# nanoporetech/tombo

Hardware: NVIDIA H100
Metric: resquiggle_reads_per_sec (higher is better)
Workload: dtype f64

## Files before the change

### include/tombo_b200.h

```cpp
#ifndef TOMBO_B200_H
#define TOMBO_B200_H
#include <stdint.h>

#ifdef __cplusplus
extern "C" {
#endif

#define TB2_ABI_VERSION 1

enum {
    TB2_OK = 0,
    TB2_ERR_FEWER_CPTS = 1,
    TB2_ERR_BEYOND_BANDWIDTH = 2,
    TB2_ERR_ADAPTIVE_BEYOND_SIGNAL = 3,
    TB2_ERR_NOT_ENOUGH_DEL_SIGNAL = 4,
    TB2_ERR_TOO_MANY_DELS = 5,
    TB2_ERR_INVALID_SEG = 6,
    TB2_ERR_ZERO_LEN_SEG = 7,
    TB2_ERR_NEG_SEG = 8,
    TB2_ERR_SEG_PAST_END = 9,
    TB2_ERR_START_TOO_FAR = 10,
    TB2_ERR_MASKED_TOO_FEW = 11,
    TB2_ERR_READ_TOO_SHORT_START = 12,
    TB2_ERR_MAP_TOO_SHORT_START = 13,
    TB2_ERR_POOR_START_MATCH = 14,
    TB2_ERR_DISCORDANT_LEN = 15,
    TB2_ERR_OPEN_PORE = 16,
    TB2_ERR_NO_RAW = 17,
    TB2_ERR_TOO_MUCH_SIGNAL = 18,
    TB2_ERR_SEG_COUNT = 19,
    TB2_ERR_THEIL_SEN_ZERO = 20,
    TB2_ERR_INVALID_START_PATH = 21,
    TB2_ERR_UNEXPECTED = 100,
    TB2_ERR_CUDA = 200,
    TB2_ERR_INVALID_ARG = 201,
    TB2_ERR_CAPACITY = 202,
    TB2_ERR_INVALID_SEQ = 203
};

typedef struct tb2_params {
    double match_evalue, skip_pen;
    int64_t bandwidth;
    double max_half_z_score;
    int64_t running_stat_width, min_obs_per_base, raw_min_obs_per_base,
        mean_obs_per_event;
    double z_shift, stay_pen;
    int64_t use_t_test_seg;
    int64_t band_bound_thresh, start_bw, start_save_bw, start_n_bases;
} tb2_params;

typedef struct tb2_scale_values {
    double shift, scale, lower_lim, upper_lim, outlier_thresh;
} tb2_scale_values;

typedef struct tb2_policy {
    double outlier_thresh;
    int64_t max_raw_cpts;
    double min_event_to_seq_ratio;
    double sig_match_thresh;
    int64_t max_scaling_iters;
    int64_t is_rna;
    int64_t skip_seq_scaling;
    double const_scale;
    uint32_t subsample_seed;
    uint32_t rescue;
} tb2_policy;

typedef struct tb2_ctx tb2_ctx;

int tb2_abi_version(void);
int tb2_device_count(void);
int tb2_ctx_create(int device, tb2_ctx **out);
void tb2_ctx_destroy(tb2_ctx *ctx);
const char *tb2_status_message(int status);
const char *tb2_last_error(tb2_ctx *ctx);
int64_t tb2_launch_count(tb2_ctx *ctx);
int tb2_last_timing(tb2_ctx *ctx, double *out4);

void *tb2_host_alloc(size_t bytes);
void tb2_host_free(void *p);

int tb2_set_model(tb2_ctx *ctx, const double *means, const double *sds,
                  int kmer_width, int central_pos);
int tb2_set_alt_model(tb2_ctx *ctx, const double *alt_means, int kmer_width);

int tb2_new_means(tb2_ctx *ctx, const double *sig, int64_t n_sig,
                  const int64_t *segs, int64_t n_segs, double *means_out);
int tb2_new_mean_stds(tb2_ctx *ctx, const double *sig, int64_t n_sig,
                      const int64_t *segs, int64_t n_segs, double *means_out,
                      double *sds_out);
int tb2_normalize_raw_signal(tb2_ctx *ctx, const double *raw, int64_t n,
                             int norm_type, double outlier_thresh,
                             double const_scale, const tb2_scale_values *sv_in,
                             double *norm_out, tb2_scale_values *sv_out);
int tb2_identify_stalls(tb2_ctx *ctx, const double *raw, int64_t n, int64_t *ints_out,
                        int64_t cap, int64_t *n_out);
int tb2_valid_cpts_w_cap(tb2_ctx *ctx, const double *sig, int64_t n,
                         int64_t min_base_obs, int64_t running_stat_width,
                         int64_t num_cpts, int t_test, int64_t *cpts_out,
                         int *read_status);
int tb2_banded_forward_pass(tb2_ctx *ctx, const double *z,
                            const int64_t *event_starts, int64_t n_bases,
                            int64_t bw, double skip_pen, double stay_pen,
                            double *fwd_out, int64_t *tb_out);
int tb2_banded_traceback(tb2_ctx *ctx, const int64_t *tb,
                         const int64_t *event_starts, int64_t n_bases,
                         int64_t bw, int64_t band_pos,
                         int64_t band_boundary_thresh, int64_t *seq_poss_out,
                         int *read_status);
int tb2_adaptive_banded_forward_pass(
    tb2_ctx *ctx, double *fwd, int64_t *tb, int64_t *event_starts,
    int64_t n_bases, int64_t bw, const double *event_means, int64_t n_events,
    const double *ref_means, const double *ref_sds, double z_shift,
    double skip_pen, double stay_pen, int64_t start_seq_pos,
    double mask_fill_z_score, int do_winsorize_z, double max_half_z_score,
    int *read_status);
int tb2_theil_sen(tb2_ctx *ctx, double prev_shift, double prev_scale,
                  const double *event_means, const double *model_means,
                  int64_t n, uint32_t subsample_key, double *out4,
                  int *read_status);

int tb2_find_adaptive_base_assignment(
    tb2_ctx *ctx, const int64_t *valid_cpts, int64_t n_cpts,
    const double *event_means, const tb2_params *params,
    const double *ref_means, const double *ref_sds, int64_t n_bases,
    double sig_match_thresh, int64_t *segs_out, int64_t *read_start_rel_to_raw,
    int64_t *dbg, int *read_status);
int tb2_find_static_base_assignment(tb2_ctx *ctx, const double *event_means,
                                    int64_t n_events, const double *ref_means,
                                    const double *ref_sds, int64_t n_bases,
                                    const tb2_params *params, int64_t *read_tb_out,
                                    int *read_status);
int tb2_find_seq_start_in_events(tb2_ctx *ctx, const double *event_means,
                                 int64_t n_events, const double *ref_means,
                                 const double *ref_sds, int64_t n_ref,
                                 const tb2_params *params, int64_t num_bases,
                                 int64_t num_events, int check_score,
                                 double sig_match_thresh, int64_t *start_loc,
                                 double *events_per_base, int *read_status);
int tb2_debug_last_assignment(tb2_ctx *ctx, int64_t n_bases, int64_t *starts_out,
                              int64_t *read_tb_out);
int tb2_debug_div_check(tb2_ctx *ctx, uint64_t seed, int blocks, int per_thread,
                        uint64_t *mismatches, double *example4);
int tb2_debug_counters(tb2_ctx *ctx, unsigned long long *out8, int reset);
int tb2_resolve_skipped_bases_with_raw(
    tb2_ctx *ctx, const int64_t *segs, int64_t n_bases, const double *ref_means,
    const double *ref_sds, const double *norm_signal, int64_t n_norm,
    const tb2_params *params, int64_t max_raw_cpts, int64_t *segs_out,
    int *read_status);

int tb2_resquiggle_batch(
    tb2_ctx *ctx, int64_t n_reads, const void *raw, int raw_dtype,
    const int64_t *raw_off, const uint8_t *seq, const int64_t *seq_off,
    const tb2_params *params, const tb2_params *save_params,
    const tb2_policy *policy, int64_t *segs, int64_t *read_start_rel_to_raw,
    tb2_scale_values *scale_out, double *sig_match_score, double *norm_mean,
    double *norm_signal, int32_t *status, int32_t *n_iters, int32_t *flags);

int tb2_pipeline_chunks(int sm_count, int64_t n_reads, int64_t *starts_out, int cap);

int tb2_batch_upload(tb2_ctx *ctx, int64_t n_reads, const void *raw, int raw_dtype,
                     const int64_t *raw_off, const uint8_t *seq,
                     const int64_t *seq_off, const tb2_params *params,
                     const tb2_policy *policy);
int tb2_batch_set_read_inputs(tb2_ctx *ctx, const tb2_scale_values *sv_in,
                              const int64_t *stall_ints, const int64_t *stall_off);
int tb2_batch_compute(tb2_ctx *ctx, const tb2_params *params,
                      const tb2_params *save_params, const tb2_policy *policy,
                      int want_norm_signal);
int tb2_batch_download(tb2_ctx *ctx, int64_t *segs, int64_t *read_start_rel_to_raw,
                       tb2_scale_values *scale_out, double *sig_match_score,
                       double *norm_mean, double *norm_signal, int32_t *status,
                       int32_t *n_iters, int32_t *flags);

int tb2_alt_model_llr_batch(
    tb2_ctx *ctx, int64_t n_reads, const double *norm_mean,
    const int64_t *mean_off, const uint8_t *seq, const int64_t *seq_off,
    const int64_t *read_start, int alt_base_code, int use_standard_llhr,
    double scale_factor, double height_factor, double height_power,
    double *llr_out, int64_t *pos_out, int64_t *site_off);

int tb2_calc_llh_ratio_windows(tb2_ctx *ctx, int mode, int64_t n_sites, int kmer_width,
                               const double *means, const double *ref_means,
                               const double *alt_means, const double *var_a,
                               const double *var_b, double scale_factor,
                               double height_factor, double height_power,
                               double *llr_out);

int tb2_timer_start(tb2_ctx *ctx);
int tb2_timer_stop(tb2_ctx *ctx, double *ms_out);

int tb2_batch_alt_llr(tb2_ctx *ctx, const int64_t *read_start, int alt_base_code,
                      int use_standard_llhr, double scale_factor, double height_factor,
                      double height_power, int64_t *n_sites_total);
int tb2_batch_llr_download(tb2_ctx *ctx, double *llr_out, int64_t *pos_out, int64_t *site_off);

int tb2_region_stats_begin(tb2_ctx *ctx, int64_t reg_start, int64_t reg_len);
int tb2_region_stats_add(tb2_ctx *ctx, int64_t n, const double *stats, const int64_t *pos,
                         double single_read_thresh, double lower_thresh, int stat_type);
int tb2_region_stats_add_batch_llr(tb2_ctx *ctx, double single_read_thresh,
                                   double lower_thresh, int stat_type);
int tb2_region_counts_get(tb2_ctx *ctx, int32_t *counts);
int tb2_region_counts_set(tb2_ctx *ctx, const int32_t *counts);
int tb2_region_stats_finalize(tb2_ctx *ctx, double unmod_count, double mod_count, int64_t cap,
                              int64_t *pos_out, double *frac_out, double *damp_frac_out,
                              int64_t *cov_out, int64_t *valid_cov_out, int64_t *n_out);

int tb2_window_fisher_pvals(tb2_ctx *ctx, int64_t n_segs, const double *means,
                            const double *ref_means, const double *ref_sds,
                            const int64_t *seg_off, int64_t fm_offset, int final_clamp,
                            double *pvals_out);
int tb2_de_novo_read_stats_batch(tb2_ctx *ctx, int64_t n_reads, const double *norm_mean,
                                 const int64_t *mean_off, const uint8_t *seq,
                                 const int64_t *seq_off, const int64_t *read_start,
                                 int64_t fm_offset, double *pvals_out, int64_t *pos_out,
                                 int64_t *stat_off);

int tb2_group_reg_stats(tb2_ctx *ctx, int64_t reg_start, int64_t reg_len,
                        int64_t n_samp, const double *samp_levels, const int64_t *samp_off,
                        const int64_t *samp_start, int64_t n_ctrl, const double *ctrl_levels,
                        const int64_t *ctrl_off, const int64_t *ctrl_start, int test,
                        int return_stat, int64_t min_test_reads, int64_t fm_offset, int64_t cap,
                        int64_t *pos_out, double *stat_out, int64_t *cov_out,
                        int64_t *ctrl_cov_out, int64_t *n_out);
int tb2_reads_ref_levels(tb2_ctx *ctx, int64_t reg_start, int64_t reg_len, int64_t n_reads,
                         const double *levels, const int64_t *off, const int64_t *start,
                         int64_t min_test_reads, int est_mean, const double *prior_means,
                         const double *prior_sds, double mean_prior_weight,
                         double sd_prior_weight, double *means_out, double *sds_out,
                         int64_t *cov_out);

#ifdef __cplusplus
}
#endif
#endif
```

### tombo_b200/csrc/stage_kernels.cu

```cuda
#include "stage_kernels.cuh"

static inline int grid1d(int n, int bs) { return (n + bs - 1) / bs; }

int tb2_launch_prep(tb2_ctx *ctx, const BatchView &b, const void *raw_dev, int raw_dtype,
                    int is_rna, long long, long long)
{
    if (raw_dtype == 0)
        k_prep<double><<<b.n_reads, ST_THREADS, 0, ctx->stream>>>(
            b, (const double *)raw_dev, is_rna, ctx->model_means.as<double>(),
            ctx->model_sds.as<double>());
    else
        k_prep<short><<<b.n_reads, ST_THREADS, 0, ctx->stream>>>(
            b, (const short *)raw_dev, is_rna, ctx->model_means.as<double>(),
            ctx->model_sds.as<double>());
    TB2_CHECK_LAUNCH(ctx);
    return TB2_OK;
}

int tb2_launch_start_attempt(tb2_ctx *ctx, const BatchView &b, int attempt)
{
    k_start_attempt<<<grid1d(b.n_reads, 256), 256, 0, ctx->stream>>>(b, attempt);
    TB2_CHECK_LAUNCH(ctx);
    return TB2_OK;
}

int tb2_launch_begin_call(tb2_ctx *ctx, const BatchView &b, const tb2_params &p,
                          const StagePolicy &pol)
{
    k_begin_call<<<grid1d(b.n_reads, 256), 256, 0, ctx->stream>>>(b, p, pol);
    TB2_CHECK_LAUNCH(ctx);
    return TB2_OK;
}

int tb2_launch_end_call(tb2_ctx *ctx, const BatchView &b, int max_iters)
{
    k_end_call<<<grid1d(b.n_reads, 256), 256, 0, ctx->stream>>>(b, max_iters);
    TB2_CHECK_LAUNCH(ctx);
    return TB2_OK;
}

int tb2_launch_count_active(tb2_ctx *ctx, const BatchView &b, int *dev_counter)
{
    TB2_CUDA_TRY(ctx, cudaMemsetAsync(dev_counter, 0, 2 * sizeof(int), ctx->stream));
    k_count_active<<<grid1d(b.n_reads, 256), 256, 0, ctx->stream>>>(b, dev_counter);
    TB2_CHECK_LAUNCH(ctx);
    return TB2_OK;
}

int tb2_launch_normalize(tb2_ctx *ctx, const BatchView &b, const StagePolicy &pol, int first_call)
{
    k_normalize<<<b.n_reads, ST_THREADS, 0, ctx->stream>>>(b, pol, first_call);
    TB2_CHECK_LAUNCH(ctx);
    return TB2_OK;
}

int tb2_launch_cpts(tb2_ctx *ctx, const BatchView &b, const tb2_params &p, int on_raw)
{
    if (!p.use_t_test_seg) {
        k_cumsum<<<(b.n_reads + CS_WARPS - 1) / CS_WARPS, CS_WARPS * 32, 0, ctx->stream>>>(b, on_raw);
        TB2_CHECK_LAUNCH(ctx);
    }
    const long long nw = (b.max_raw + 32) / 32;
    long long words = (4 + std::max(0, (int)p.min_obs_per_base - 1)) * nw;
    if (words * 4 > 48 * 1024) words = 0;
    k_cpts<<<b.n_reads, ST_THREADS, (size_t)words * 4, ctx->stream>>>(b, p, on_raw, (int)words);
    TB2_CHECK_LAUNCH(ctx);
    return TB2_OK;
}

int tb2_launch_rna_scale(tb2_ctx *ctx, const BatchView &b, const StagePolicy &pol)
{
    k_rna_scale<<<b.n_reads, ST_THREADS, 0, ctx->stream>>>(b, pol);
    TB2_CHECK_LAUNCH(ctx);
    return TB2_OK;
}

int tb2_launch_event_means(tb2_ctx *ctx, const BatchView &b)
{
    k_event_means<<<b.n_reads, ST_THREADS, 0, ctx->stream>>>(b);
    TB2_CHECK_LAUNCH(ctx);
    return TB2_OK;
}

int tb2_launch_stalls(tb2_ctx *ctx, const BatchView &b)
{
    k_stalls<<<b.n_reads, ST_THREADS, 0, ctx->stream>>>(b);
    TB2_CHECK_LAUNCH(ctx);
    return TB2_OK;
}

int tb2_launch_resolve(tb2_ctx *ctx, const BatchView &b, const tb2_params &p,
                       const StagePolicy &pol, size_t cap)
{
    enum { SLOT_RAWDP = 73, SLOT_CNT2 = 74, SLOT_RAWBIG = 75 };
    const int warps_per_block = 4;
    int grid = ctx->sm_count * 8;
    const int max_useful = (b.n_reads + warps_per_block - 1) / warps_per_block;
    if (grid > max_useful) grid = max_useful > 0 ? max_useful : 1;
    const size_t slots = (size_t)grid * warps_per_block;
    TB2_CUDA_TRY(ctx, ctx->pool[SLOT_RAWDP].reserve(slots * cap * sizeof(double)));
    TB2_CUDA_TRY(ctx, ctx->pool[SLOT_CNT2].reserve(16));
    TB2_CUDA_TRY(ctx, cudaMemsetAsync(ctx->pool[SLOT_CNT2].p, 0, 16, ctx->stream));
    const unsigned long long big_cap = std::min<unsigned long long>(
        (2ULL << 30) / 8, std::max<unsigned long long>((64ULL << 20) / 8, 24ULL * 64ULL * (unsigned long long)std::max(1, b.max_raw)));
    TB2_CUDA_TRY(ctx, ctx->pool[SLOT_RAWBIG].reserve((size_t)big_cap * sizeof(double)));
    k_resolve<<<grid, warps_per_block * 32, 0, ctx->stream>>>(
        b, p, pol, ctx->pool[SLOT_RAWDP].as<double>(), cap, ctx->pool[SLOT_CNT2].as<int>(),
        ctx->pool[SLOT_RAWBIG].as<double>(), big_cap,
        (unsigned long long *)(ctx->pool[SLOT_CNT2].as<int>() + 2));
    TB2_CHECK_LAUNCH(ctx);
    return TB2_OK;
}

int tb2_launch_base_means(tb2_ctx *ctx, const BatchView &b)
{
    k_base_means<<<b.n_reads, ST_THREADS, 0, ctx->stream>>>(b);
    TB2_CHECK_LAUNCH(ctx);
    return TB2_OK;
}

int tb2_launch_theil_sen(tb2_ctx *ctx, const BatchView &b, const StagePolicy &pol, int first_call)
{
    const size_t smem = sizeof(TsSmem);
    TB2_CUDA_TRY(ctx, cudaFuncSetAttribute(k_theil_sen, cudaFuncAttributeMaxDynamicSharedMemorySize,
                                           (int)smem));
    k_theil_sen<<<b.n_reads, ST_THREADS, smem, ctx->stream>>>(b, pol, first_call);
    TB2_CHECK_LAUNCH(ctx);
    return TB2_OK;
}

int tb2_launch_finalize(tb2_ctx *ctx, const BatchView &b, const StagePolicy &pol, int first_call,
                        double *norm_mean_out, double *norm_signal_out)
{
    k_finalize<<<b.n_reads, ST_THREADS, 0, ctx->stream>>>(b, pol, first_call, norm_mean_out,
                                                          norm_signal_out);
    TB2_CHECK_LAUNCH(ctx);
    return TB2_OK;
}

extern "C" int tb2_debug_counters(tb2_ctx *ctx, unsigned long long *out8, int reset)
{
    int rc = tb2_use(ctx);
    if (rc) return rc;
    if (!out8) return TB2_ERR_INVALID_ARG;
    TB2_CUDA_TRY(ctx, cudaStreamSynchronize(ctx->stream));
    TB2_CUDA_TRY(ctx, cudaMemcpyFromSymbol(out8, g_tb2_counters, 64));
    if (reset) {
        unsigned long long z[8] = {0};
        TB2_CUDA_TRY(ctx, cudaMemcpyToSymbol(g_tb2_counters, z, 64));
    }
    return TB2_OK;
}
```

### tombo_b200/csrc/stage_kernels.cuh

```cuda
#pragma once
#include "batch.h"
#include "select.cuh"

#define ST_THREADS TB2_SEL_THREADS

__device__ __forceinline__ bool rd_active(const ReadState &s) { return s.active && s.status == TB2_OK; }

template <class T>
__global__ void __launch_bounds__(ST_THREADS)
k_prep(BatchView b, const T *raw, int is_rna, const double *kmeans, const double *ksds)
{
    const int r = blockIdx.x;
    const long long ro = b.raw_off[r];
    const int n = (int)(b.raw_off[r + 1] - ro);
    for (int i = threadIdx.x; i < n; i += ST_THREADS)
        b.rawf[ro + i] = (double)raw[ro + (is_rna ? n - 1 - i : i)];
    const long long so = b.seq_off[r], bo = b.base_off[r];
    const int nb = (int)(b.base_off[r + 1] - bo);
    const int K = b.kmer_width;
    int bad = 0;
    for (int i = threadIdx.x; i < nb; i += ST_THREADS) {
        int code = 0;
        for (int j = 0; j < K; ++j) {
            const int c = b.seq[so + i + j];
// ... 692 lines not shown
        for (int i = lane; i <= nb; i += 32) out[i] = segs[i];
        __syncwarp();
        const int n_norm = segs[nb];
        if (lane == 0) s.n_norm = n_norm;
        const double *norm = b.norm + b.raw_off[r] + s.rsrtr;
        const double *rm = b.rm + bo, *rs = b.rs + bo;
        int *ws = b.starts + bo, *we = b.read_tb + bo + r;
        const int n_segs = nb + 1;
        const int m = (int)p.raw_min_obs_per_base;
        int nw = 0, st = TB2_OK;
#define TOO_SMALL(a, z) ((double)(segs[z] - segs[a]) <= ((double)(((z) - (a) + 1) * m)) * EXTRA_SIG_FACTOR)
#define MERGE_TRIM() do { \
            int mm = 0; \
            for (int k = 0; k < nw; ++k) { \
                if (mm > 0 && ws[k] < we[mm - 1]) we[mm - 1] = we[k]; \
                else { ws[mm] = ws[k]; we[mm] = we[k]; ++mm; } } \
            nw = mm; \
            if (ws[0] < 0) ws[0] = 0; \
            if (we[nw - 1] > n_segs - 1) we[nw - 1] = n_segs - 1; } while (0)
        if (lane == 0) {
            for (int d = 0; d < nb; ++d) {
                if (segs[d + 1] - segs[d] != 0) continue;
                if (nw > 0 && d < we[nw - 1] + DEL_FIX_WINDOW) we[nw - 1] = d + DEL_FIX_WINDOW + 1;
                else { ws[nw] = d - DEL_FIX_WINDOW; we[nw] = d + DEL_FIX_WINDOW + 1; ++nw; }
            }
            if (nw > 0) {
                MERGE_TRIM();
                int expanded = 0;
                for (int it = 0; it < MAX_DEL_FIX_WINDOW - DEL_FIX_WINDOW; ++it) {
                    expanded = 0;
                    for (int k = 0; k < nw; ++k)
                        if (TOO_SMALL(ws[k], we[k])) { expanded = 1; ws[k] -= 1; we[k] += 1; }
                    if (!expanded) break;
                    MERGE_TRIM();
                }
                if (expanded)
                    for (int k = 0; k < nw; ++k)
                        if (TOO_SMALL(ws[k], we[k])) { st = TB2_ERR_NOT_ENOUGH_DEL_SIGNAL; break; }
                if (st == TB2_OK && pol.max_raw_cpts >= 0) {
                    int mx = 0;
                    for (int k = 0; k < nw; ++k) mx = max(mx, we[k] - ws[k]);
                    if (mx > pol.max_raw_cpts) st = TB2_ERR_TOO_MANY_DELS;
                }
            }
        }
        nw = __shfl_sync(TB2_FULL_MASK, nw, 0);
        st = __shfl_sync(TB2_FULL_MASK, st, 0);
        if (nw == 0) continue;
        __syncwarp();
        for (int k = 0; k < nw && st == TB2_OK; ++k) {
            const int a = ws[k], z = we[k], n_ev = z - a;
            const int sig_start = segs[a], sig_len = segs[z] - segs[a];
            if (sig_start < 0 || sig_start + sig_len > n_norm) { st = TB2_ERR_UNEXPECTED; break; }
            RawCtx c;
            c.sig = norm + sig_start; c.rm = rm + a; c.rs = rs + a;
            c.n_ev = n_ev; c.m = m;
            c.L = sig_len - (n_ev - 1) * m;
            c.winsor = !isnan(p.max_half_z_score);
            c.mhz = c.winsor ? p.max_half_z_score : 0.0;
            if (c.L < 1) { st = TB2_ERR_UNEXPECTED; break; }
            const size_t need = (size_t)n_ev * c.L + 3 * (size_t)c.L + 8;
            unsigned long long woff = 0;
            if (need > cap) {
                if (lane == 0) woff = atomicAdd(big_used, (unsigned long long)need) + 1ULL;
                woff = __shfl_sync(TB2_FULL_MASK, woff, 0);
                if (woff - 1ULL + need > big_cap) { st = TB2_ERR_CAPACITY; break; }
            }
            double *win = woff ? big_pool + (woff - 1ULL) : scr;
            c.fwd = win;
            c.cs = win + (size_t)n_ev * c.L;
            c.ld0 = (int *)(c.cs + 2 * (size_t)c.L);
            c.ld1 = c.ld0 + c.L;
            if (n_ev < 2) { st = TB2_ERR_UNEXPECTED; break; }
            if (m == 1) raw_forward_wf(c);
            else raw_fill_z(c);
            if (lane == 0) {
                st = (m == 1) ? TB2_OK : raw_window(c, out + a + 1);
                if (st == TB2_OK) st = raw_traceback_rows(c, out + a + 1);
                if (st == TB2_OK) for (int i = 0; i < n_ev - 1; ++i) out[a + 1 + i] += sig_start;
            }
            st = __shfl_sync(TB2_FULL_MASK, st, 0);
            __syncwarp();
        }
        if (lane != 0) continue;
        if (st == TB2_OK) {
            for (int i = 0; i < nb; ++i) if (out[i + 1] - out[i] < 1) { st = TB2_ERR_ZERO_LEN_SEG; break; }
            if (st == TB2_OK && out[0] < 0) st = TB2_ERR_NEG_SEG;
            if (st == TB2_OK && out[nb] > n_norm) st = TB2_ERR_SEG_PAST_END;
        }
        if (st != TB2_OK) s.status = st;
    }
}

__global__ void __launch_bounds__(ST_THREADS) k_base_means(BatchView b)
{
    const int r = blockIdx.x;
    const ReadState &s = b.st[r];
    if (!rd_active(s)) return;
    const long long bo = b.base_off[r];
    const int nb = (int)(b.base_off[r + 1] - bo);
    const double *norm = b.norm + b.raw_off[r] + s.rsrtr;
    const int *segs = b.segs + bo + r;
    for (int i = threadIdx.x; i < nb; i += ST_THREADS) {
        const int a = segs[i], z = segs[i + 1];
        double acc = 0;
        for (int k = a; k < z; ++k) acc += norm[k];
        b.bm[bo + i] = acc / (double)(z - a);
    }
}

__device__ unsigned long long g_tb2_counters[8];

#define TS_MAX 1000
#define TS_BINS 2048
#define TS_BUF 2048

#define TS_ABINS 4096

#define TS_PAD 1024

struct TsSmem {
    double ev[TS_PAD], md[TS_PAD];
    float4 pt[TS_PAD];
    union {
        unsigned int hist[TS_ABINS + 2];
        double buf[TS_BUF];
    };
    unsigned int nbuf, nout, b1, b2, below, maxabs_bits;
    int ok;
};

__device__ __forceinline__ double ts_slope(const TsSmem &t, int i, int j)
{
    return (t.ev[i] == t.ev[j]) ? 1000.0 : (t.md[i] - t.md[j]) / (t.ev[i] - t.ev[j]);
}

template <class Fn>
__device__ __forceinline__ void ts_for_pairs(int n, Fn fn)
{
    const int half = (n + 1) / 2;
    for (int c = threadIdx.x; c < half; c += ST_THREADS) {
        const int j0 = c, j1 = n - 1 - c;
        for (int i = 0; i < j0; ++i) fn(i, j0);
        if (j1 != j0) for (int i = 0; i < j1; ++i) fn(i, j1);
    }
}

template <class Fn>
__device__ __forceinline__ void ts_for_cols(int n, Fn fn)
{
    const int half = (n + 1) / 2;
    for (int c = threadIdx.x; c < half; c += ST_THREADS) {
        const int j0 = c, j1 = n - 1 - c;
        fn(j0);
        if (j1 != j0) fn(j1);
    }
}

__device__ __forceinline__ void ts_pair_of(long long s, int n, int *pi, int *pj)
{
    double disc = (double)(2 * n - 1) * (double)(2 * n - 1) - 8.0 * (double)s;
    int i = (int)(((double)(2 * n - 1) - sqrt(disc)) / 2.0);
    if (i < 0) i = 0;
    auto row_start = [&](int q) { return (long long)q * (2 * n - q - 1) / 2; };
    while (i > 0 && row_start(i) > s) --i;
    while (row_start(i + 1) <= s) ++i;
    *pi = i;
    *pj = (int)(s - row_start(i)) + i + 1;
}


#define TS_SBINS 1024
#define TS_SAMPLES 2048
#define TS_LIST 4096
#define TS_MAX_PHASES 600

__device__ long long ts_sort_count(double **ka, double **kb, unsigned short **pa, unsigned short **pb,
                                   int P, SelectSmem &sm)
{
    const int tid = threadIdx.x;
    unsigned int inv = 0;
    for (int w = 1; w < P; w <<= 1) {
        const double *src = *ka; const unsigned short *sp = *pa;
        double *dst = *kb; unsigned short *dp = *pb;
        for (int p = tid; p < P; p += ST_THREADS) {
            const int base = p & ~(2 * w - 1), mid = base + w;
            const double key = src[p];
            int lo, hi;
            if (p < mid) {
                lo = mid; hi = mid + w;
                while (lo < hi) { const int m = (lo + hi) >> 1; if (src[m] < key) lo = m + 1; else hi = m; }
                dst[p + (lo - mid)] = key; dp[p + (lo - mid)] = sp[p];
            } else {
                lo = base; hi = mid;
                while (lo < hi) { const int m = (lo + hi) >> 1; if (src[m] <= key) lo = m + 1; else hi = m; }
                const int le = lo - base;
                dst[base + (p - mid) + le] = key; dp[base + (p - mid) + le] = sp[p];
                inv += (unsigned int)(w - le);
            }
        }
        __syncthreads();
        double *tk = *ka; *ka = *kb; *kb = tk;
        unsigned short *tp = *pa; *pa = *pb; *pb = tp;
    }
    return (long long)tb2_block_sum(inv, sm);
}

__device__ long long ts_sweep(unsigned short *perm, const double *q, int n, unsigned int *list,
                              unsigned int *n_list, SelectSmem &sm)
{
    const int tid = threadIdx.x;
    unsigned int swaps = 0;
    int quiet = 0;
    for (int ph = 0; ph < TS_MAX_PHASES; ++ph) {
        int any = 0;
        for (int p = 2 * tid + (ph & 1); p + 1 < n; p += 2 * ST_THREADS) {
            const unsigned short x = perm[p], y = perm[p + 1];
            if (q[x] > q[y]) {
                perm[p] = y; perm[p + 1] = x;
                ++swaps; any = 1;
                if (list) {
                    const unsigned int slot = atomicAdd(n_list, 1u);
                    if (slot < TS_LIST) list[slot] = ((unsigned int)min(x, y) << 16) | (unsigned int)max(x, y);
                }
            }
        }
        any = __syncthreads_or(any);
        quiet = any ? 0 : quiet + 1;
        if (quiet >= 2) {
#ifdef TS_DEBUG
            if (tid == 0) atomicAdd(&g_tb2_counters[7], (unsigned long long)(ph + 1));
#endif
            return (long long)tb2_block_sum(swaps, sm);
        }
    }
    tb2_block_sum(swaps, sm);
    return -1;
}

__device__ bool ts_gaps_ok(const unsigned short *perm, const double *q, const double *ev, int n, double g)
{
    int bad = 0;
    for (int p = threadIdx.x; p + 1 < n; p += ST_THREADS) {
        const int x = perm[p], y = perm[p + 1];
        bad |= !(q[y] - q[x] > g) && (ev[x] != ev[y]);
    }
    return !__syncthreads_or(bad);
}

__global__ void __launch_bounds__(ST_THREADS, 4)
k_theil_sen(BatchView b, StagePolicy pol, int first_call)
{
    TB2_DYN_SMEM(unsigned char, ts_raw);
    TsSmem &t = *reinterpret_cast<TsSmem *>(ts_raw);
    __shared__ SelectSmem sm;
    const int r = b.order ? b.order[blockIdx.x] : blockIdx.x;
    ReadState &s = b.st[r];
    if (!rd_active(s)) return;
    const int tid = threadIdx.x;
    if (first_call && pol.skip_seq_scaling) {
        if (tid == 0) { s.changed = 0; s.shc = 0.0; s.scc = 1.0; }
        return;
    }
    const long long bo = b.base_off[r];
    const int nb = (int)(b.base_off[r + 1] - bo);
    const double *bm = b.bm + bo, *rm = b.rm + bo;
    int n = nb;
    if (nb > TS_MAX) {
        n = TS_MAX;
        const unsigned int key = pol.literal_key
            ? pol.subsample_seed
            : tb2_subsample_key(pol.subsample_seed, (unsigned int)(r + pol.read_index_base),
                                (unsigned int)s.calls);
        for (int i = tid; i < n; i += ST_THREADS) {
            const int k = tb2_perm_index(i, nb, key);
            t.ev[i] = bm[k]; t.md[i] = rm[k];
        }
    } else {
        for (int i = tid; i < n; i += ST_THREADS) { t.ev[i] = bm[i]; t.md[i] = rm[i]; }
    }
    __syncthreads();
    const long long Np = (long long)n * (n - 1) / 2;
    if (Np <= 0) { if (tid == 0) s.status = TB2_ERR_UNEXPECTED; return; }
    if (tid == 0) atomicAdd(&g_tb2_counters[0], 1ULL);
    const bool even = (Np % 2) == 0;
    const long long k1 = even ? Np / 2 - 1 : Np / 2;
    double v1 = 0, v2 = 0;
    bool have = false;
    const int hs = n / 2;
    double lo = 0, hi = 0;
    if (hs >= 16) {
        for (int i = tid; i < hs; i += ST_THREADS) t.buf[i] = ts_slope(t, i, i + hs);
        __syncthreads();
        double d0;
        auto f_samp = [&](int i) { return t.buf[i]; };
        tb2_block_select2(f_samp, PredAll(), hs, (int)(hs * 0.30), false, &lo, &d0, sm);
        tb2_block_select2(f_samp, PredAll(), hs, (int)(hs * 0.70), false, &hi, &d0, sm);
    }
    {
        int P = 2;
        while (P < n) P <<= 1;
        for (int i = n + tid; i < P; i += ST_THREADS) { t.ev[i] = __longlong_as_double(0x7ff0000000000000LL); t.md[i] = 0.0; }
        __syncthreads();
        for (int k = 2; k <= P; k <<= 1) {
            for (int jj = k >> 1; jj > 0; jj >>= 1) {
                for (int idx = tid; idx < (P >> 1); idx += ST_THREADS) {
                    const int a = ((idx & ~(jj - 1)) << 1) | (idx & (jj - 1)), c = a | jj;
                    const double ea = t.ev[a], ec = t.ev[c];
                    const double ma = t.md[a], mc = t.md[c];
                    const bool gt = (ea > ec) || (ea == ec && ma > mc);
                    const bool ne = (ea != ec) || (ma != mc);
                    if (ne && (gt == ((a & k) == 0))) {
                        t.ev[a] = ec; t.ev[c] = ea;
                        t.md[a] = mc; t.md[c] = ma;
                    }
                }
                __syncthreads();
            }
        }
    }
    if (hs >= 16 && n >= 128 && hi > lo && hi < 1000.0) {
        double *qa = reinterpret_cast<double *>(t.pt), *qb = qa + TS_PAD;
        unsigned short *pa = reinterpret_cast<unsigned short *>(t.buf + (TS_BUF - 512)), *pb = pa + TS_PAD;
        unsigned int *list = reinterpret_cast<unsigned int *>(qb);
        static_assert(TS_LIST * 4 <= TS_PAD * 8 + (TS_BUF - 512) * 8, "pair list overlaps the id arrays");
        bool ok;
        double M;
        const int n_samples = (int)min(8192LL, max(2048LL, Np / 24));
        {
            int bad = 0;
            double mx = 0.0;
            for (int i = tid; i < n; i += ST_THREADS) {
                const double e = t.ev[i], m = t.md[i];
                if (!(fabs(e) < 1e300) || !(fabs(m) < 1e300)) bad = 1;
                if (i + 1 < n && !(t.ev[i + 1] >= e)) bad = 1;
                mx = fmax(mx, fmax(fabs(e), fabs(m)));
            }
            ok = !__syncthreads_or(bad);
#ifdef TS_DEBUG
            if (!ok && tid == 0) { int c = 0; for (int i = 0; i + 1 < n; ++i) if (!(t.ev[i + 1] > t.ev[i])) { if (c++ < 3) printf("  ev order: i=%d %.17g %.17g\n", i, t.ev[i], t.ev[i + 1]); } }
#endif
            unsigned long long mk = (unsigned long long)__double_as_longlong(mx);
            mk = ~tb2_block_min_u64(~mk, sm);
            M = fmax(1.0, __longlong_as_double((long long)mk));
        }
        const float lo_f = (float)lo, hi_f = (float)hi;
        const float w_f = (hi_f - lo_f) / (float)TS_SBINS;
        ok = ok && (w_f > 0.0f) && isfinite(w_f);
        if (ok) {
            for (int i = tid; i < TS_SBINS + 2; i += ST_THREADS) t.hist[i] = 0;
            __syncthreads();
            const float inv_w = 1.0f / w_f;
            for (int q = tid; q < n_samples; q += ST_THREADS) {
                const uint32_t h1 = tb2_mix32((uint32_t)q * 2654435761u + 17u), h2 = tb2_mix32(h1 ^ 0x9E3779B9u);
                const int i = (int)(((unsigned long long)h1 * (unsigned long long)n) >> 32);
                int j = i + 1 + (int)(((unsigned long long)h2 * (unsigned long long)(n - 1)) >> 32);
                if (j >= n) j -= n;
                const double de = t.ev[i] - t.ev[j];
                const float sa = __fdividef((float)(t.md[i] - t.md[j]), (float)de);
                int bin = 0;
                if (sa >= hi_f || de == 0.0) bin = TS_SBINS + 1;
                else if (sa >= lo_f) bin = min(TS_SBINS - 1, (int)((sa - lo_f) * inv_w)) + 1;
                atomicAdd(&t.hist[bin], 1u);
            }
            __syncthreads();
            const int per = (TS_SBINS + 2 + ST_THREADS - 1) / ST_THREADS;
            const int q0 = min(TS_SBINS + 2, tid * per), q1 = min(TS_SBINS + 2, q0 + per);
            unsigned int mine = 0;
            for (int q = q0; q < q1; ++q) mine += t.hist[q];
            const int lane = tid & 31, warp = tid >> 5;
            unsigned int inc = mine;
#pragma unroll
            for (int off = 1; off < 32; off <<= 1) {
                const unsigned int o = __shfl_up_sync(TB2_FULL_MASK, inc, off);
                if (lane >= off) inc += o;
            }
            if (lane == 31) sm.warp_tot[warp] = inc;
            __syncthreads();
            unsigned int run = inc - mine;
            for (int q = 0; q < warp; ++q) run += sm.warp_tot[q];
            for (int q = q0; q < q1; ++q) { run += t.hist[q]; t.hist[q] = run; }
            __syncthreads();
        }
        auto pick = [&](double frac, int *bsel) -> bool {
            const double tf = frac * (double)n_samples;
            if (!(tf > (double)t.hist[0]) || !(tf < (double)t.hist[TS_SBINS])) return false;
            const unsigned int target = (unsigned int)tf;
            int blo = 1, bhi = TS_SBINS;
            while (blo < bhi) { const int m = (blo + bhi) >> 1; if (t.hist[m] >= target) bhi = m; else blo = m + 1; }
            *bsel = blo;
            return true;
        };
        auto thr = [&](int bsel) { return (double)lo_f + (double)w_f * (double)bsel; };
        const long long kT = even ? k1 + 1 : k1;
        const double sig = 0.5 / sqrt((double)n_samples);
        const double ppm = (double)Np / (double)n_samples;
        int bL = 0, bH1 = 0, bH2 = 0;
        long long invL = 0, inv1 = 0, inv2 = 0;
        if (ok) ok = pick((double)k1 / (double)Np - 3.0 * sig, &bL);
        if (ok) {
            const double TL = thr(bL);
            const double gL = 1e-12 * M * (1.0 + fabs(TL));
            int P = 2;
            while (P < n) P <<= 1;
            for (int i = tid; i < P; i += ST_THREADS) {
                qa[i] = (i < n) ? __fma_rn(-TL, t.ev[i], t.md[i]) : __longlong_as_double(0x7ff0000000000000LL);
                pa[i] = (unsigned short)i;
            }
            __syncthreads();
            double *ka = qa, *kb = qb;
            unsigned short *ia = pa, *ib = pb;
            invL = ts_sort_count(&ka, &kb, &ia, &ib, P, sm);
            int bad = 0;
            for (int p2 = tid; p2 + 1 < n; p2 += ST_THREADS)
                bad |= !(ka[p2 + 1] - ka[p2] > gL) && (t.ev[ia[p2]] != t.ev[ia[p2 + 1]]);
            ok = !__syncthreads_or(bad);
            if (ia != pa) for (int i = tid; i < n; i += ST_THREADS) pa[i] = ia[i];
            __syncthreads();
            ok = ok && invL <= k1;
        }
        bH1 = bL; inv1 = invL;
        for (int stage = 0; ok && stage < 5; ++stage) {
            const double D = (double)(k1 - inv1);
            const double rest = fmax(3.0 * sqrt(D * ppm), 150.0);
            if (D <= rest + 250.0 || D + 3.0 * sqrt(D * ppm) + 300.0 <= 0.8 * TS_LIST) break;
            const double delta = (double)inv1 / (double)Np - (double)t.hist[bH1] / (double)n_samples;
            int bn;
            if (!pick(((double)k1 - rest) / (double)Np - delta, &bn) || bn <= bH1) break;
            const double T1 = thr(bn);
            for (int i = tid; i < n; i += ST_THREADS) qa[i] = __fma_rn(-T1, t.ev[i], t.md[i]);
            __syncthreads();
            const long long sw = ts_sweep(pa, qa, n, nullptr, nullptr, sm);
            ok = sw >= 0 && ts_gaps_ok(pa, qa, t.ev, n, 1e-12 * M * (1.0 + fabs(T1)));
            bH1 = bn; inv1 += sw;
            ok = ok && inv1 <= k1;
#ifdef TS_DEBUG
            if (tid == 0) printf("  stage %d: D=%.0f aimed rest %.0f -> got rest %lld (swaps %lld)\n", stage, D, rest, k1 - inv1, sw);
#endif
        }
        if (ok) {
            const double D = (double)(kT - inv1);
            const double over = fmax(3.0 * sqrt(fmax(D, 1.0) * ppm), 150.0);
            const double delta = (double)inv1 / (double)Np - (double)t.hist[bH1] / (double)n_samples;
            ok = pick(((double)kT + over) / (double)Np - delta, &bH2) && bH2 > bH1;
            if (ok) {
                const double T2 = thr(bH2);
                for (int i = tid; i < n; i += ST_THREADS) qa[i] = __fma_rn(-T2, t.ev[i], t.md[i]);
                if (tid == 0) t.nbuf = 0;
                __syncthreads();
                const long long sw = ts_sweep(pa, qa, n, list, &t.nbuf, sm);
                ok = sw >= 0 && sw <= TS_LIST && ts_gaps_ok(pa, qa, t.ev, n, 1e-12 * M * (1.0 + fabs(T2)));
                inv2 = inv1 + sw;
                ok = ok && kT < inv2;
            }
        }
        if (ok) {
            const int K = (int)(inv2 - inv1);
            __syncthreads();
            double mine_v[TS_LIST / ST_THREADS];
#pragma unroll
            for (int u = 0; u < TS_LIST / ST_THREADS; ++u) {
                const int q = tid + u * ST_THREADS;
                mine_v[u] = 0.0;
                if (q < K) {
                    const int i = (int)(list[q] >> 16), j = (int)(list[q] & 0xffffu);
                    mine_v[u] = (t.md[i] - t.md[j]) / (t.ev[i] - t.ev[j]);
                }
            }
            __syncthreads();
            double *outv = reinterpret_cast<double *>(t.pt);
#pragma unroll
            for (int u = 0; u < TS_LIST / ST_THREADS; ++u) {
                const int q = tid + u * ST_THREADS;
                if (q < K) outv[q] = mine_v[u];
            }
            __syncthreads();
            tb2_block_select2([&](int i) { return outv[i]; }, PredAll(), K, (int)(k1 - inv1), even,
                              &v1, &v2, sm);
            have = true;
            if (tid == 0) atomicAdd(&g_tb2_counters[5], 1ULL);
        } else if (tid == 0) {
            atomicAdd(&g_tb2_counters[6], 1ULL);
#ifdef TS_DEBUG
            printf("ts abandon: n=%d Np=%lld k1=%lld bL=%d bH1=%d bH2=%d invL=%lld inv1=%lld inv2=%lld nbuf=%u cum0=%u cumN=%u\n", n, Np, k1, bL, bH1, bH2, invL, inv1, inv2, t.nbuf, t.hist[0], t.hist[TS_SBINS]);
#endif
        }
        __syncthreads();
    }
    if (!have && hs >= 16 && Np > 4 * TS_ABINS) {
        const float lo_f = (float)lo, hi_f = (float)hi;
        const float w_f = (hi_f - lo_f) / (float)TS_ABINS;
        if (hi_f > lo_f && w_f > 0.0f && isfinite(w_f)) {
            const float inv_w = 1.0f / w_f;
            if (tid == 0) t.maxabs_bits = 0u;
            __syncthreads();
            {
                float mx = 0.0f;
                for (int i = tid; i < n; i += ST_THREADS)
                    mx = fmaxf(mx, fmaxf(fabsf((float)t.ev[i]), fabsf((float)t.md[i])));
                if (!(mx < 3.0e38f)) mx = 3.0e38f;
                atomicMax(&t.maxabs_bits, __float_as_uint(mx));
            }
            int stride = (int)min(8LL, max(1LL, 518400LL / Np));
            for (; !have && stride >= 1; stride = (stride > 1) ? 1 : 0) {
                for (int i = tid; i < n; i += ST_THREADS)
                    t.pt[i] = make_float4((float)t.ev[i], (float)t.md[i], 0.0f, 0.0f);
                for (int i = tid; i < TS_ABINS + 2; i += ST_THREADS) t.hist[i] = 0;
                if (tid == 0) { t.nbuf = 0; t.ok = 0; t.below = 0; t.b1 = 0; t.b2 = 0; }
                __syncthreads();
                unsigned int n_under = 0, n_smp = 0;
                ts_for_cols(n, [&](int j) {
                    const float4 pj = t.pt[j];
                    const int jm = j % stride;
                    int i = jm ? stride - jm : 0;
                    for (; i < j; i += stride) {
                        const float4 pi = t.pt[i];
                        const float de = pi.x - pj.x;
                        float sa = __fdividef(pi.y - pj.y, de);
                        if (de == 0.0f) sa = 1000.0f;
                        ++n_smp;
                        n_under += sa < lo_f;
                        if (sa >= lo_f && sa < hi_f)
                            atomicAdd(&t.hist[min(TS_ABINS - 1, (int)((sa - lo_f) * inv_w)) + 1], 1u);
                    }
                });
                n_under = tb2_block_sum(n_under, sm);
                n_smp = tb2_block_sum(n_smp, sm);
                if (tid == 0) t.hist[0] = n_under;
                __syncthreads();
                long long kA, kB;
                if (stride == 1) { kA = k1; kB = even ? k1 + 1 : k1; }
                else {
                    const long long kS = (long long)((double)k1 * (double)n_smp / (double)Np);
                    const long long mg = (long long)(1.25 * sqrt((double)n_smp)) + 2;
                    kA = kS - mg; kB = kS + mg;
                }
                if (tid == 0) { t.b1 = 0; t.b2 = TS_ABINS + 1; }
                __syncthreads();
                if (kA >= 0 && kB < (long long)n_smp) {
                    const int per = (TS_ABINS + 2 + ST_THREADS - 1) / ST_THREADS;
                    const int q0 = min(TS_ABINS + 2, tid * per), q1 = min(TS_ABINS + 2, q0 + per);
                    unsigned int mine = 0;
                    for (int q = q0; q < q1; ++q) mine += t.hist[q];
                    const int lane = tid & 31, warp = tid >> 5;
                    unsigned int inc = mine;
#pragma unroll
                    for (int off = 1; off < 32; off <<= 1) {
                        const unsigned int o = __shfl_up_sync(TB2_FULL_MASK, inc, off);
                        if (lane >= off) inc += o;
                    }
                    if (lane == 31) sm.warp_tot[warp] = inc;
                    __syncthreads();
                    unsigned int base = 0;
                    for (int q = 0; q < warp; ++q) base += sm.warp_tot[q];
                    long long cum = (long long)base + inc - mine;
                    for (int q = q0; q < q1; ++q) {
                        const long long c = t.hist[q];
                        if (kA >= cum && kA < cum + c) t.b1 = q;
                        if (kB >= cum && kB < cum + c) t.b2 = q;
                        cum += c;
                    }
                }
                __syncthreads();
                const int bA = (int)t.b1, bB = (int)t.b2;
                if (bA >= 1 && bB <= TS_ABINS && bA <= bB) {
                    const double L = (double)lo_f + (double)w_f * (double)(bA - 2);
                    const double H = (double)lo_f + (double)w_f * (double)(bB + 1);
                    const float M = fmaxf(1.0f, __uint_as_float(t.maxabs_bits));
                    const float Lf = (float)L, Hf = (float)H;
                    const float gLf = 1e-5f * M * (1.0f + fabsf(Lf)), gHf = 1e-5f * M * (1.0f + fabsf(Hf));
                    __syncthreads();
                    for (int i = tid; i < n; i += ST_THREADS) {
                        const float ef = t.pt[i].x, mf = t.pt[i].y;
                        t.pt[i] = make_float4(fmaf(-Lf, ef, mf), fmaf(-Hf, ef, mf), ef, 0.0f);
                    }
                    __syncthreads();
                    unsigned int below = 0;
                    unsigned int *queue = reinterpret_cast<unsigned int *>(t.buf);
                    const unsigned int QCAP = 2 * TS_BUF;
                    auto push = [&](int i, int j) {
                        const unsigned int slot = atomicAdd(&t.nbuf, 1u);
                        if (slot < QCAP) queue[slot] = ((unsigned int)i << 16) | (unsigned int)j;
                    };
                    {
                        const int half = (n + 1) / 2;
                        for (int cidx = tid; cidx < half; cidx += ST_THREADS) {
                            const int ja = cidx, jb = n - 1 - cidx;
                            const float4 pa = t.pt[ja], pb = t.pt[jb];
                            const float xla = pa.x + gLf, yha = pa.y - gHf;
                            const float xlb = pb.x + gLf, yhb = pb.y - gHf;
                            int i = 0;
                            if (ja != jb) {
#pragma unroll 4
                                for (; i < ja; ++i) {
                                    const float4 pi = t.pt[i];
                                    const bool la = pi.x > xla, ha = pi.y < yha;
                                    const bool lb = pi.x > xlb, hb = pi.y < yhb;
                                    if ((la || ha) && pi.z != pa.z) below += la; else push(i, ja);
                                    if ((lb || hb) && pi.z != pb.z) below += lb; else push(i, jb);
                                }
                            }
#pragma unroll 4
                            for (; i < jb; ++i) {
                                const float4 pi = t.pt[i];
                                const bool lb = pi.x > xlb, hb = pi.y < yhb;
                                if ((lb || hb) && pi.z != pb.z) below += lb; else push(i, jb);
                            }
                        }
                    }
                    __syncthreads();
                    const unsigned int nq = t.nbuf;
                    double *outv = reinterpret_cast<double *>(t.pt);
                    if (tid == 0) t.nout = 0;
                    __syncthreads();
                    if (nq <= QCAP) {
                        for (unsigned int q = tid; q < nq; q += ST_THREADS) {
                            const int i = (int)(queue[q] >> 16), j = (int)(queue[q] & 0xffffu);
                            const double de = t.ev[i] - t.ev[j], dm = t.md[i] - t.md[j];
                            const double sv = (de == 0.0) ? 1000.0 : dm / de;
                            if (sv < L) ++below;
                            else if (sv < H) {
// ... 124 lines not shown
```

Baseline: 577,200.

## Run small-stride bitonic sort phases in registers with warp shuffles

For Theil-Sen bitonic sorts whose padded size fits in one block (64 to 2*ST_THREADS), each thread keeps two elements in registers. Phases with stride below 64 are done with __shfl_xor_sync exchanges instead of shared-memory passes separated by __syncthreads. Larger strides still go through shared memory. The aim is to cut block-wide barriers and shared-memory traffic in the sort. A profiling script and an occupancy debug entry point are also added. Inactive threads skip the shuffles while the full mask is used, which is only safe if every active warp is fully populated.

```diff
diff --git a/include/tombo_b200.h b/include/tombo_b200.h
--- a/include/tombo_b200.h
+++ b/include/tombo_b200.h
@@ -143,6 +143,7 @@
 int tb2_debug_div_check(tb2_ctx *ctx, uint64_t seed, int blocks, int per_thread,
                         uint64_t *mismatches, double *example4);
 int tb2_debug_counters(tb2_ctx *ctx, unsigned long long *out8, int reset);
+int tb2_debug_theil_sen_occupancy(tb2_ctx *ctx, int *out2);
 int tb2_resolve_skipped_bases_with_raw(
     tb2_ctx *ctx, const int64_t *segs, int64_t n_bases, const double *ref_means,
     const double *ref_sds, const double *norm_signal, int64_t n_norm,
diff --git a/profile_stages.py b/profile_stages.py
--- /dev/null
+++ b/profile_stages.py
@@ -0,0 +1,151 @@
+#!/usr/bin/env python
+import argparse
+import ctypes as C
+import json
+import os
+import re
+import subprocess
+import sys
+
+import numpy as np
+
+REPO = os.path.dirname(os.path.abspath(__file__))
+sys.path.insert(0, REPO)
+
+import bench
+
+
+def gpu_info(device):
+    import torch
+    info = {'name': torch.cuda.get_device_name(device), 'power_limit_w': None, 'sm_max_mhz': None}
+    try:
+        import pynvml as nv
+        nv.nvmlInit()
+        h = nv.nvmlDeviceGetHandleByIndex(device)
+        info['power_limit_w'] = nv.nvmlDeviceGetPowerManagementLimit(h) / 1000.0
+        info['sm_max_mhz'] = nv.nvmlDeviceGetMaxClockInfo(h, nv.NVML_CLOCK_SM)
+    except Exception:
+        try:
+            o = subprocess.run(['nvidia-smi', '-i', str(device), '--query-gpu=power.limit,clocks.max.sm',
+                                '--format=csv,noheader,nounits'], capture_output=True, text=True,
+                               timeout=10).stdout.strip().split(',')
+            info['power_limit_w'], info['sm_max_mhz'] = float(o[0]), float(o[1])
+        except Exception:
+            pass
+    return info
+
+
+def theil_sen_occupancy(ctx):
+    fn = ctx.lib.tb2_debug_theil_sen_occupancy
+    fn.restype = C.c_int
+    out = (C.c_int * 2)()
+    ctx.check(fn(ctx.handle, out))
+    return {'ctas_per_sm': out[0], 'smem_bytes': out[1]}
+
+
+def counters(ctx, reset):
+    fn = ctx.lib.tb2_debug_counters
+    fn.restype = C.c_int
+    out = (C.c_uint64 * 8)()
+    ctx.check(fn(ctx.handle, out, C.c_int(int(reset))))
+    return list(out)
+
+
+def kernel_name(name):
+    name = re.sub(r'^void\s+', '', name)
+    depth, out = 0, []
+    for ch in name:
+        if ch == '(' and depth == 0:
+            break
+        depth += ch == '<'
+        depth -= ch == '>'
+        out.append(ch)
+    return ''.join(out).strip()
+
+
+def main():
+    ap = argparse.ArgumentParser()
+    ap.add_argument('--reads', type=int, default=bench.CONFIGS['c1']['reads'])
+    ap.add_argument('--steps', type=int, default=3, help='profiled steps')
+    ap.add_argument('--warmup', type=int, default=2)
+    ap.add_argument('--round-raw', action='store_true',
+                    help='round the signal to integers (the int16 DAC case)')
+    ap.add_argument('--out', default='profile_stages_out', help='directory for the trace')
+    ap.add_argument('--device', type=int, default=0)
+    args = ap.parse_args()
+
+    import torch
+    from torch.profiler import ProfilerActivity, profile
+    from tombo_b200 import _lib, synthetic as syn
+
+    cfg = bench.CONFIGS['c1']
+    kmer_ref, cpos, raw, raw_off, seq, seq_off = bench.make_workload(cfg, args.reads, 1)
+    if args.round_raw:
+        np.round(raw, out=raw)
+    k = len(kmer_ref[0][0])
+    means, sds = syn.kmer_table(kmer_ref)
+    nb = (seq_off[1:] - seq_off[:-1]) - (k - 1)
+    torch.cuda.init()
+    ctx = _lib.Context(args.device)
+    ctx.set_model(means, sds, k, cpos)
+    rp = bench.RP(cfg['aln'], cfg['seg'])
+    sp = bench.RP(cfg['aln'], cfg['seg'], save=True)
+    pol = _lib.make_policy(cfg['kind'], subsample_seed=0)
+    ctx.batch_upload(raw, raw_off, seq, seq_off, rp, pol)
+    for _ in range(args.warmup):
+        ctx.batch_compute(rp, sp, pol)
+    step_ms = []
+    for _ in range(args.steps):
+        ctx.timer_start()
+        ctx.batch_compute(rp, sp, pol)
+        step_ms.append(ctx.timer_stop())
+    counters(ctx, 1)
+    ctx.batch_compute(rp, sp, pol)
+    cnt = counters(ctx, 1)
+    torch.cuda.synchronize()
+    with profile(activities=[ProfilerActivity.CUDA]) as prof:
+        for _ in range(args.steps):
+            ctx.batch_compute(rp, sp, pol)
+        torch.cuda.synchronize()
+    tot, calls = {}, {}
+    for e in prof.events():
+        if e.device_type != torch.autograd.DeviceType.CUDA:
+            continue
+        n = kernel_name(e.name)
+        tot[n] = tot.get(n, 0.0) + (e.time_range.end - e.time_range.start) / 1e3
+        calls[n] = calls.get(n, 0) + 1
+    all_ms = sum(tot.values())
+    os.makedirs(args.out, exist_ok=True)
+    trace = os.path.join(args.out, 'profile_stages%s.pt.trace.json' % ('_round' if args.round_raw else ''))
+    prof.export_chrome_trace(trace)
+
+    res = {'gpu': gpu_info(args.device), 'reads': args.reads, 'round_raw': bool(args.round_raw),
+           'max_bases': int(nb.max()),
+           'step_ms_events': step_ms, 'step_ms_kernels': all_ms / args.steps,
+           'theil_sen_occupancy': theil_sen_occupancy(ctx),
+           'counters_per_step': {'theil_sen_reads': cnt[0], 'sort_and_sweep': cnt[5],
+                                 'abandoned_sort_and_sweep': cnt[6], 'all': cnt},
+           'kernels': {}}
+    g = res['gpu']
+    print('GPU %s, power limit %s W, max SM clock %s MHz' % (g['name'], g['power_limit_w'], g['sm_max_mhz']))
+    print('%d reads%s, step %.2f ms (CUDA events, median of %d), kernel time %.2f ms / step'
+          % (args.reads, ' (rounded signal)' if args.round_raw else '', float(np.median(step_ms)),
+             len(step_ms), all_ms / args.steps))
+    print('%-44s %10s %9s %7s' % ('kernel', 'ms/step', 'launches', 'share'))
+    for n in sorted(tot, key=lambda x: -tot[x]):
+        ms = tot[n] / args.steps
+        res['kernels'][n] = {'ms_per_step': ms, 'launches_per_step': calls[n] / args.steps,
+                             'share': tot[n] / all_ms}
+        print('%-44s %10.3f %9.1f %6.1f%%' % (n[:44], ms, calls[n] / args.steps, 100.0 * tot[n] / all_ms))
+    ts = sum(v['ms_per_step'] for n, v in res['kernels'].items() if n.startswith('k_theil_sen'))
+    res['theil_sen_ms_per_step'] = ts
+    print('Theil-Sen (all launches): %.3f ms / step' % ts)
+    print('occupancy:', res['theil_sen_occupancy'])
+    print('counters per step: %d Theil-Sen reads, %d sort-and-sweep, %d abandoned'
+          % (cnt[0], cnt[5], cnt[6]))
+    print(json.dumps(res))
+    ctx.close()
+
+
+if __name__ == '__main__':
+    main()
diff --git a/tombo_b200/csrc/stage_kernels.cu b/tombo_b200/csrc/stage_kernels.cu
--- a/tombo_b200/csrc/stage_kernels.cu
+++ b/tombo_b200/csrc/stage_kernels.cu
@@ -151,3 +151,17 @@
     }
     return TB2_OK;
 }
+
+extern "C" int tb2_debug_theil_sen_occupancy(tb2_ctx *ctx, int *out2)
+{
+    int rc = tb2_use(ctx);
+    if (rc) return rc;
+    if (!out2) return TB2_ERR_INVALID_ARG;
+    const size_t smem = sizeof(TsSmem);
+    TB2_CUDA_TRY(ctx, cudaFuncSetAttribute(k_theil_sen, cudaFuncAttributeMaxDynamicSharedMemorySize,
+                                           (int)smem));
+    TB2_CUDA_TRY(ctx, cudaOccupancyMaxActiveBlocksPerMultiprocessor(&out2[0], k_theil_sen,
+                                                                    ST_THREADS, smem));
+    out2[1] = (int)smem;
+    return TB2_OK;
+}
diff --git a/tombo_b200/csrc/stage_kernels.cuh b/tombo_b200/csrc/stage_kernels.cuh
--- a/tombo_b200/csrc/stage_kernels.cuh
+++ b/tombo_b200/csrc/stage_kernels.cuh
@@ -1018,21 +1018,59 @@
         while (P < n) P <<= 1;
         for (int i = n + tid; i < P; i += ST_THREADS) { t.ev[i] = __longlong_as_double(0x7ff0000000000000LL); t.md[i] = 0.0; }
         __syncthreads();
-        for (int k = 2; k <= P; k <<= 1) {
-            for (int jj = k >> 1; jj > 0; jj >>= 1) {
-                for (int idx = tid; idx < (P >> 1); idx += ST_THREADS) {
-                    const int a = ((idx & ~(jj - 1)) << 1) | (idx & (jj - 1)), c = a | jj;
-                    const double ea = t.ev[a], ec = t.ev[c];
-                    const double ma = t.md[a], mc = t.md[c];
-                    const bool gt = (ea > ec) || (ea == ec && ma > mc);
-                    const bool ne = (ea != ec) || (ma != mc);
-                    if (ne && (gt == ((a & k) == 0))) {
-                        t.ev[a] = ec; t.ev[c] = ea;
-                        t.md[a] = mc; t.md[c] = ma;
+        auto swaps = [](int a, int k, double ea, double ma, double ec, double mc) {
+            const bool gt = (ea > ec) || (ea == ec && ma > mc);
+            const bool ne = (ea != ec) || (ma != mc);
+            return ne && (gt == ((a & k) == 0));
+        };
+        auto smem_phase = [&](int k, int jj) {
+            for (int idx = tid; idx < (P >> 1); idx += ST_THREADS) {
+                const int a = ((idx & ~(jj - 1)) << 1) | (idx & (jj - 1)), c = a | jj;
+                const double ea = t.ev[a], ec = t.ev[c];
+                const double ma = t.md[a], mc = t.md[c];
+                if (swaps(a, k, ea, ma, ec, mc)) {
+                    t.ev[a] = ec; t.ev[c] = ea;
+                    t.md[a] = mc; t.md[c] = ma;
+                }
+            }
+            __syncthreads();
+        };
+        if (P >= 64 && P <= 2 * ST_THREADS) {
+            const bool act = tid < (P >> 1);
+            double e0 = 0, e1 = 0, m0 = 0, m1 = 0;
+            auto load = [&]() { e0 = t.ev[2 * tid]; e1 = t.ev[2 * tid + 1]; m0 = t.md[2 * tid]; m1 = t.md[2 * tid + 1]; };
+            auto store = [&]() { t.ev[2 * tid] = e0; t.ev[2 * tid + 1] = e1; t.md[2 * tid] = m0; t.md[2 * tid + 1] = m1; };
+            auto xchg = [&](int i, int k, int jj, double &e, double &m) {
+                const double eo = __shfl_xor_sync(TB2_FULL_MASK, e, jj >> 1);
+                const double mo = __shfl_xor_sync(TB2_FULL_MASK, m, jj >> 1);
+                const bool lower = (i & jj) == 0;
+                if (lower ? swaps(i, k, e, m, eo, mo) : swaps(i & ~jj, k, eo, mo, e, m)) { e = eo; m = mo; }
+            };
+            if (act) load();
+            for (int k = 2; k <= P; k <<= 1) {
+                int jj = k >> 1;
+                if (jj >= 64) {
+                    if (act) store();
+                    __syncthreads();
+                    for (; jj >= 64; jj >>= 1) smem_phase(k, jj);
+                    if (act) load();
+                }
+                if (act) {
+                    for (; jj >= 2; jj >>= 1) {
+                        xchg(2 * tid, k, jj, e0, m0);
+                        xchg(2 * tid + 1, k, jj, e1, m1);
+                    }
+                    if (swaps(2 * tid, k, e0, m0, e1, m1)) {
+                        const double te = e0, tm = m0;
+                        e0 = e1; m0 = m1; e1 = te; m1 = tm;
                     }
                 }
-                __syncthreads();
-            }
+            }
+            if (act) store();
+            __syncthreads();
+        } else {
+            for (int k = 2; k <= P; k <<= 1)
+                for (int jj = k >> 1; jj > 0; jj >>= 1) smem_phase(k, jj);
         }
     }
     if (hs >= 16 && n >= 128 && hi > lo && hi < 1000.0) {
```

After: 579,300, median of 6. No clear change (+0.3%).
